# gwall-ceres/HighRes-net

Hardware: AMD Instinct MI355X
Metric: SR frames/sec (384x384 out) at B=32, n_views=32 (higher is better)
Workload: dtype bf16

## Files before the change

### highres-net_amd/hrnet_hip/csrc/common.h

```cpp
#pragma once
#include <hip/hip_runtime.h>
#include <stdint.h>
#include <stddef.h>
#include "prof.h"

#define HRN_F32 0
#define HRN_BF16 1
#define HRN_BF16X3 2

typedef __attribute__((ext_vector_type(8))) __bf16 bf16x8;
typedef __attribute__((ext_vector_type(4))) float f32x4;
typedef __attribute__((ext_vector_type(16))) float f32x16;
typedef __attribute__((ext_vector_type(4))) unsigned u32x4;
typedef __attribute__((ext_vector_type(2))) unsigned u32x2;

void hrn_set_error(const char* fmt, ...);
int hrn_allow_lds(const void* kernel, int bytes);
int hrn_device_cus(void);
#define HRN_CHECK(cond, code, ...)                                \
    do {                                                          \
        if (!(cond)) { hrn_set_error(__VA_ARGS__); return (code); } \
    } while (0)
#define HRN_HIP(call)                                                                    \
    do {                                                                                 \
        hipError_t e_ = (call);                                                          \
        if (e_ != hipSuccess) {                                                          \
            hrn_set_error("%s failed: %s (%s:%d)", #call, hipGetErrorString(e_), __FILE__, __LINE__); \
            return -5;                                                                   \
        }                                                                                \
    } while (0)
#define HRN_LAUNCH_CHECK()  HRN_HIP(hipGetLastError())

__device__ __forceinline__ float bf16_bits_to_f32(unsigned short b) {
    return __uint_as_float(((unsigned)b) << 16);
}
__device__ __forceinline__ unsigned short f32_to_bf16_bits(float f) {
    __bf16 h = (__bf16)f;
    return __builtin_bit_cast(unsigned short, h);
}
__device__ __forceinline__ unsigned pack2_bf16(float lo, float hi) {
    typedef __bf16 bf16x2_t __attribute__((ext_vector_type(2)));
    typedef float f32x2_t __attribute__((ext_vector_type(2)));
    const f32x2_t v = {lo, hi};
    return __builtin_bit_cast(unsigned, __builtin_convertvector(v, bf16x2_t));
}
__device__ __forceinline__ void split2_bf16(float a, float b, unsigned& hi, unsigned& lo) {
    hi = pack2_bf16(a, b);
    lo = pack2_bf16(a - __uint_as_float(hi << 16), b - __uint_as_float(hi & 0xffff0000u));
}

__device__ __forceinline__ void quad_transpose(u32x4 (&x)[4], bool b0, bool b1) {
#pragma unroll
    for (int d = 0; d < 4; ++d) {
#pragma unroll
        for (int p = 0; p < 4; p += 2) {
            const unsigned a = x[p][d], b = x[p + 1][d];
            const unsigned ra = (unsigned)__builtin_amdgcn_update_dpp(0, (int)b, 0xB1, 0xF, 0xF, true);
            const unsigned rb = (unsigned)__builtin_amdgcn_update_dpp(0, (int)a, 0xB1, 0xF, 0xF, true);
            x[p][d] = b0 ? ra : a;
            x[p + 1][d] = b0 ? b : rb;
        }
#pragma unroll
        for (int p = 0; p < 2; ++p) {
            const unsigned a = x[p][d], b = x[p + 2][d];
            const unsigned ra = (unsigned)__builtin_amdgcn_update_dpp(0, (int)b, 0x4E, 0xF, 0xF, true);
            const unsigned rb = (unsigned)__builtin_amdgcn_update_dpp(0, (int)a, 0x4E, 0xF, 0xF, true);
            x[p][d] = b1 ? ra : a;
            x[p + 2][d] = b1 ? b : rb;
        }
    }
}

template <int DT> struct ElemOf;
template <> struct ElemOf<HRN_F32>  { typedef float type;          static constexpr int size = 4; };
template <> struct ElemOf<HRN_BF16> { typedef unsigned short type; static constexpr int size = 2; };

template <int DT> __device__ __forceinline__ float load_elem(const void* p, size_t i);
template <> __device__ __forceinline__ float load_elem<HRN_F32>(const void* p, size_t i) { return ((const float*)p)[i]; }
template <> __device__ __forceinline__ float load_elem<HRN_BF16>(const void* p, size_t i) { return bf16_bits_to_f32(((const unsigned short*)p)[i]); }

template <int DT> __device__ __forceinline__ void store_elem(void* p, size_t i, float v);
template <> __device__ __forceinline__ void store_elem<HRN_F32>(void* p, size_t i, float v) { ((float*)p)[i] = v; }
template <> __device__ __forceinline__ void store_elem<HRN_BF16>(void* p, size_t i, float v) { ((unsigned short*)p)[i] = f32_to_bf16_bits(v); }

template <int DT> __device__ __forceinline__ f32x4 load4(const void* p, size_t i);
template <> __device__ __forceinline__ f32x4 load4<HRN_F32>(const void* p, size_t i) {
    return *(const f32x4*)((const float*)p + i);
}
template <> __device__ __forceinline__ f32x4 load4<HRN_BF16>(const void* p, size_t i) {
    uint2 u = *(const uint2*)((const unsigned short*)p + i);
    f32x4 r;
    r[0] = __uint_as_float(u.x << 16); r[1] = __uint_as_float(u.x & 0xffff0000u);
    r[2] = __uint_as_float(u.y << 16); r[3] = __uint_as_float(u.y & 0xffff0000u);
    return r;
}
template <int DT> __device__ __forceinline__ void store4(void* p, size_t i, f32x4 v);
template <> __device__ __forceinline__ void store4<HRN_F32>(void* p, size_t i, f32x4 v) {
    *(f32x4*)((float*)p + i) = v;
}
template <> __device__ __forceinline__ void store4<HRN_BF16>(void* p, size_t i, f32x4 v) {
    uint2 u; u.x = pack2_bf16(v[0], v[1]); u.y = pack2_bf16(v[2], v[3]);
    *(uint2*)((unsigned short*)p + i) = u;
}

template <int ST> __device__ __forceinline__ f32x4 act_ld4(const void* p, size_t lo, size_t i4) {
    if constexpr (ST == HRN_BF16X3) {
        const u32x2 h = __builtin_nontemporal_load((const u32x2*)p + i4);
        const u32x2 l = __builtin_nontemporal_load((const u32x2*)((const unsigned char*)p + lo) + i4);
        f32x4 r;
        r[0] = __uint_as_float(h[0] << 16) + __uint_as_float(l[0] << 16);
        r[1] = __uint_as_float(h[0] & 0xffff0000u) + __uint_as_float(l[0] & 0xffff0000u);
        r[2] = __uint_as_float(h[1] << 16) + __uint_as_float(l[1] << 16);
        r[3] = __uint_as_float(h[1] & 0xffff0000u) + __uint_as_float(l[1] & 0xffff0000u);
        return r;
    } else if constexpr (ST == HRN_BF16) {
        const u32x2 h = __builtin_nontemporal_load((const u32x2*)p + i4);
        return f32x4{__uint_as_float(h[0] << 16), __uint_as_float(h[0] & 0xffff0000u), __uint_as_float(h[1] << 16),
                     __uint_as_float(h[1] & 0xffff0000u)};
    } else {
        static_assert(ST == HRN_F32, "storage kind");
        return __builtin_nontemporal_load((const f32x4*)p + i4);
    }
}
template <int ST> __device__ __forceinline__ void act_st4(void* p, size_t lo, size_t i4, f32x4 v) {
    if constexpr (ST == HRN_BF16X3) {
        unsigned h0, l0, h1, l1;
        split2_bf16(v[0], v[1], h0, l0);
        split2_bf16(v[2], v[3], h1, l1);
        const u32x2 h = {h0, h1}, l = {l0, l1};
        __builtin_nontemporal_store(h, (u32x2*)p + i4);
        __builtin_nontemporal_store(l, (u32x2*)((unsigned char*)p + lo) + i4);
    } else if constexpr (ST == HRN_BF16) {
        const u32x2 h = {pack2_bf16(v[0], v[1]), pack2_bf16(v[2], v[3])};
        __builtin_nontemporal_store(h, (u32x2*)p + i4);
    } else {
        static_assert(ST == HRN_F32, "storage kind");
        __builtin_nontemporal_store(v, (f32x4*)p + i4);
    }
}
template <int ST> __device__ __forceinline__ float act_ld1(const void* p, size_t lo, size_t i) {
    if constexpr (ST == HRN_BF16X3) return bf16_bits_to_f32(((const unsigned short*)p)[i]) + bf16_bits_to_f32(((const unsigned short*)((const unsigned char*)p + lo))[i]);
    else if constexpr (ST == HRN_BF16) return bf16_bits_to_f32(((const unsigned short*)p)[i]);
    else return ((const float*)p)[i];
}

#define HRN_LAUNCH_ST(dt, KERNEL, ...)                                                                   \
    do {                                                                                                 \
        if ((dt) == HRN_BF16X3) hipLaunchKernelGGL(KERNEL<HRN_BF16X3>, __VA_ARGS__);                     \
        else if ((dt) == HRN_BF16) hipLaunchKernelGGL(KERNEL<HRN_BF16>, __VA_ARGS__);                    \
        else hipLaunchKernelGGL(KERNEL<HRN_F32>, __VA_ARGS__);                                           \
    } while (0)

__device__ __forceinline__ void block_pair_sum(const double* __restrict__ partial, int nblk, int C, double& s, double& ss) {
    __shared__ double red_ps[2][1024];
    const int c = (int)threadIdx.x % C, ph = (int)threadIdx.x / C, nph = (int)blockDim.x / C;
    double a = 0.0, b = 0.0;
#pragma unroll 4
    for (int k = ph; k < nblk; k += nph) { a += partial[((size_t)k * C + c) * 2]; b += partial[((size_t)k * C + c) * 2 + 1]; }
    red_ps[0][threadIdx.x] = a; red_ps[1][threadIdx.x] = b;
    __syncthreads();
    if (ph == 0)
        for (int k = 1; k < nph; ++k) { a += red_ps[0][k * C + c]; b += red_ps[1][k * C + c]; }
    s = a; ss = b;
}

static inline size_t hrn_align_up(size_t x, size_t a) { return (x + a - 1) / a * a; }
static inline int hrn_esize(int dt) { return dt == HRN_BF16 ? 2 : 4; }
static inline bool hrn_scale_ok(int s) { return s >= 2 && s <= 4; }
```

### highres-net_amd/hrnet_hip/csrc/conv3x3_r64.hip

```cpp
#include <type_traits>
#include "conv3x3.h"

namespace {

constexpr int HALO_H = CONV_TILE_H + 2;
constexpr int HALO_W = CONV_TILE_W + 2;
constexpr int IN_BYTES = HALO_H * HALO_W * 128;
constexpr int W_BYTES = 9 * 64 * 128;
constexpr int LDS_BYTES = W_BYTES + 2 * IN_BYTES + 256;

__device__ __forceinline__ void lds_done_then_barrier() {
    asm volatile("s_waitcnt lgkmcnt(0)" ::: "memory");
    __builtin_amdgcn_s_barrier();
    asm volatile("" ::: "memory");
}

__device__ __forceinline__ float raw_max(float a, float b) {
    float y;
    asm("v_max_f32 %0, %1, %2" : "=v"(y) : "v"(a), "v"(b));
    return y;
}

__device__ __attribute__((aligned(16))) unsigned hrn_r64_zero16[4];

template <bool RES>
__global__ __launch_bounds__(512, 2) void conv3x3_r64_kernel(const ConvParams p) {
    if (p.only_if_nonpos && p.only_if_nonpos[0] > 0.f) return;
    extern __shared__ __attribute__((aligned(16))) unsigned char smem[];
    unsigned char* w_lds = smem;
    float* bias_lds = (float*)(smem + W_BYTES + 2 * IN_BYTES);

    const int tid = threadIdx.x;
    const int lane = tid & 63;
    const int wave = __builtin_amdgcn_readfirstlane(tid >> 6);
    const int team = wave >> 2, tw = wave & 3;
    unsigned char* in_lds = smem + W_BYTES + team * IN_BYTES;
    const int r = lane & 31, hh = lane >> 5;
    const int H = p.H, W = p.W;
    const size_t hw = (size_t)H * W;
    const unsigned tiles_x = (W + CONV_TILE_W - 1) / CONV_TILE_W;
    const unsigned tiles_y = (H + CONV_TILE_H - 1) / CONV_TILE_H;
    const unsigned tiles = tiles_x * tiles_y;
    const unsigned total = tiles * (unsigned)p.M;
    const unsigned G = gridDim.x;
    const unsigned bid = blockIdx.x;
    const unsigned slot = (G & 7) == 0 ? (bid & 7) * (G >> 3) + (bid >> 3) : bid;
    if (slot >= total) return;
    const int ntl = (int)((total - slot + G - 1) / G);
    const int nmine = (ntl + 1 - team) >> 1;

    unsigned cur_m = (slot + team * G) / tiles, cur_t = (slot + team * G) - cur_m * tiles;
    const unsigned step_m = (2 * G) / tiles, step_t = 2 * G - step_m * tiles;

    {
        const u32x4* wg = (const u32x4*)p.wpk;
#pragma unroll
        for (int j = 0; j < W_BYTES / 16 / 512; ++j) {
            const int idx = tid + j * 512;
            const int row = idx >> 3, c = idx & 7;
            *(u32x4*)(w_lds + row * 128 + ((c ^ ((row >> 1) & 7)) << 4)) = wg[idx];
        }
        if (tid < 64) bias_lds[tid] = p.bias[tid];
    }

    unsigned voff[11], cm_lo = 0, cm_hi = 0;
    if (!RES) {
#pragma unroll
        for (int jj = 0; jj < 11; ++jj) {
            const int j = tw + 4 * jj;
            const int pix = j * 8 + (lane >> 3);
            const int py = pix / HALO_W, px = pix - py * HALO_W;
            voff[jj] = (unsigned)((py * W + px) * 128 + (((lane & 7) ^ ((pix >> 1) & 7)) << 4));
            unsigned cls = (py == 0 ? 1u : 0u) | (py == HALO_H - 1 ? 2u : 0u) | (px == 0 ? 4u : 0u) | (px == HALO_W - 1 ? 8u : 0u);
            if (pix >= HALO_H * HALO_W) cls = 0;
            if (jj < 8) cm_lo |= cls << (4 * jj); else cm_hi |= cls << (4 * (jj - 8));
        }
    }
    unsigned pend_F = 0;
    auto issue = [&](unsigned m, unsigned t) __attribute__((always_inline)) {
        const int ty = t / tiles_x;
        const int y0 = ty * CONV_TILE_H, x0 = (t - ty * tiles_x) * CONV_TILE_W;
        const unsigned char* base = (const unsigned char*)p.in + (size_t)m * hw * 128;
        const bool fast = !RES && y0 + CONV_TILE_H <= H && x0 + CONV_TILE_W <= W && (m > 0 || y0 > 0) &&
                          ((int)m + 1 < p.M || (size_t)(y0 + CONV_TILE_H) * W + x0 + CONV_TILE_W < hw);
        pend_F = 0;
        if (fast) {
            const unsigned char* hb = base + ((long)(y0 - 1) * W + (x0 - 1)) * 128;
#pragma unroll
            for (int jj = 0; jj < 11; ++jj) {
                const int j = tw + 4 * jj;
                if (j < 43) {
                    if (jj < 10 || j * 8 + (lane >> 3) < HALO_H * HALO_W)
                        __builtin_amdgcn_global_load_lds((const __attribute__((address_space(1))) void*)(hb + voff[jj]),
                                                         (__attribute__((address_space(3))) void*)(in_lds + j * 1024), 16, 0, 0);
                }
            }
            pend_F = (y0 == 0 ? 1u : 0u) | (y0 + CONV_TILE_H == H ? 2u : 0u) | (x0 == 0 ? 4u : 0u) | (x0 + CONV_TILE_W == W ? 8u : 0u);
            __builtin_amdgcn_sched_barrier(0);
            return;
        }
        int lq = lane;
        asm volatile("" : "+v"(lq));
#pragma unroll
        for (int jj = 0; jj < 11; ++jj) {
            const int j = tw + 4 * jj;
            if (j < 43) {
                const int pix = j * 8 + (lq >> 3);
                const int lc = (lq & 7) ^ ((pix >> 1) & 7);
                const int py = pix / HALO_W, px = pix - py * HALO_W;
                const int gy = y0 - 1 + py, gx = x0 - 1 + px;
                const bool ok = (unsigned)gy < (unsigned)H && (unsigned)gx < (unsigned)W;
                const unsigned char* src = ok ? base + (unsigned)((gy * W + gx) * 128 + lc * 16) : (const unsigned char*)hrn_r64_zero16;
                if (pix < HALO_H * HALO_W)
                    __builtin_amdgcn_global_load_lds((const __attribute__((address_space(1))) void*)src,
                                                     (__attribute__((address_space(3))) void*)(in_lds + j * 1024), 16, 0, 0);
            }
        }
        __builtin_amdgcn_sched_barrier(0);
    };
    auto fix_borders = [&]() __attribute__((always_inline)) {
        if (!RES && pend_F) {
            const unsigned fm = pend_F * 0x11111111u;
            const unsigned hit_lo = cm_lo & fm, hit_hi = cm_hi & fm;
            const u32x4 z = {0u, 0u, 0u, 0u};
#pragma unroll
            for (int jj = 0; jj < 11; ++jj) {
                const int j = tw + 4 * jj;
                if (j < 43) {
                    const unsigned h = jj < 8 ? (hit_lo >> (4 * jj)) & 15u : (hit_hi >> (4 * (jj - 8))) & 15u;
                    if (h) *(u32x4*)(in_lds + j * 1024 + lane * 16) = z;
                }
            }
        }
    };

    const bool has_slope = p.slope != nullptr;
    const float slope = has_slope ? p.slope[0] : 0.f;
    const bool slope01 = slope >= 0.f && slope <= 1.f;
    const unsigned lds0 = (unsigned)(__UINTPTR_TYPE__)(__attribute__((address_space(3))) unsigned char*)smem;
    unsigned a_off[4], a_off_hi[4], b_off[4][3];
#pragma unroll
    for (int ks = 0; ks < 4; ++ks) {
        a_off[ks] = lds0 + r * 128 + (((ks * 2 + hh) ^ ((r >> 1) & 7)) << 4);
        a_off_hi[ks] = a_off[ks] + 4 * 8192;
    }
#pragma unroll
    for (int row = 0; row < 4; ++row)
#pragma unroll
        for (int kx = 0; kx < 3; ++kx) {
            const int pix = (2 * tw + row) * HALO_W + r + kx;
            b_off[row][kx] = lds0 + (unsigned)(W_BYTES + team * IN_BYTES) + (((unsigned)pix << 7) | ((unsigned)(((pix >> 1) & 7) ^ hh) << 4));
        }

    f32x16 acc[2][2];

    auto multiply = [&]() __attribute__((always_inline)) {
#pragma unroll
        for (int cb = 0; cb < 2; ++cb)
#pragma unroll
            for (int g = 0; g < 4; ++g) {
                const f32x4 b = *(const f32x4*)(bias_lds + cb * 32 + 8 * g + 4 * hh);
#pragma unroll
                for (int j = 0; j < 4; ++j) { acc[cb][0][4 * g + j] = b[j]; acc[cb][1][4 * g + j] = b[j]; }
            }
        constexpr int NK = 36;
        bf16x8 fa[3][2], fb[3][2];
        auto rd = [&](bf16x8& dst, unsigned addr, int imm) __attribute__((always_inline)) {
            asm volatile("ds_read_b128 %0, %1 offset:%2" : "=v"(dst) : "v"(addr), "n"(imm));
        };
        auto load_part = [&](int i, int part) __attribute__((always_inline)) {
            const int s_ = i % 3, tap = i >> 2, ks = i & 3;
            const int ky = tap / 3, kx = tap - ky * 3;
            if (part < 2) {
                rd(fa[s_][part], tap < 4 ? a_off[ks] : a_off_hi[ks], (tap < 4 ? tap : tap - 4) * 8192 + part * 4096);
            } else {
                unsigned kbits = 0;
                if (ks) asm volatile("s_mov_b32 %0, %1" : "=s"(kbits) : "n"(ks << 5));
                rd(fb[s_][part - 2], b_off[part - 2 + ky][kx] ^ kbits, 0);
            }
        };
        asm volatile("s_waitcnt lgkmcnt(0)" ::: "memory");
        __builtin_amdgcn_s_setprio(3);
#pragma unroll
        for (int i = 0; i < 2; ++i)
#pragma unroll
            for (int part = 0; part < 4; ++part) load_part(i, part);
        __builtin_amdgcn_sched_barrier(0);
#pragma unroll
        for (int i = 0; i < NK; ++i) {
            const int s_ = i % 3;
            const bool more = i + 2 < NK;
            if (i < NK - 1) asm volatile("s_waitcnt lgkmcnt(5)" : "+v"(fa[s_][0]), "+v"(fb[s_][0]));
            else asm volatile("s_waitcnt lgkmcnt(1)" : "+v"(fa[s_][0]), "+v"(fb[s_][0]));
            acc[0][0] = __builtin_amdgcn_mfma_f32_32x32x16_bf16(fa[s_][0], fb[s_][0], acc[0][0], 0, 0, 0);
            if (more) load_part(i + 2, 0);
            __builtin_amdgcn_sched_barrier(0);
            if (more) asm volatile("s_waitcnt lgkmcnt(5)" : "+v"(fb[s_][1]));
            else if (i == NK - 2) asm volatile("s_waitcnt lgkmcnt(4)" : "+v"(fb[s_][1]));
            else asm volatile("s_waitcnt lgkmcnt(0)" : "+v"(fb[s_][1]));
            acc[0][1] = __builtin_amdgcn_mfma_f32_32x32x16_bf16(fa[s_][0], fb[s_][1], acc[0][1], 0, 0, 0);
            if (more) load_part(i + 2, 1);
            __builtin_amdgcn_sched_barrier(0);
            asm volatile("" : "+v"(fa[s_][1]));
            acc[1][0] = __builtin_amdgcn_mfma_f32_32x32x16_bf16(fa[s_][1], fb[s_][0], acc[1][0], 0, 0, 0);
            if (more) load_part(i + 2, 2);
            __builtin_amdgcn_sched_barrier(0);
            acc[1][1] = __builtin_amdgcn_mfma_f32_32x32x16_bf16(fa[s_][1], fb[s_][1], acc[1][1], 0, 0, 0);
            if (more) load_part(i + 2, 3);
            __builtin_amdgcn_sched_barrier(0);
        }
        __builtin_amdgcn_s_setprio(0);
    };

    u32x4 resv[2][4];
    float res_alpha = 1.f;
    auto fetch_residual = [&]() __attribute__((always_inline)) {
        const int m = (int)cur_m;
        const int ty = cur_t / tiles_x;
        const int y0 = ty * CONV_TILE_H, x0 = (cur_t - ty * tiles_x) * CONV_TILE_W;
        const unsigned char* rbase = (const unsigned char*)p.res + (size_t)m * hw * 128;
        if (p.res_mode == 3) {
            const int ob = m / p.out_h, oi = m - ob * p.out_h;
            rbase = (const unsigned char*)p.res + ((size_t)ob * p.res_vs + oi) * hw * 128;
            res_alpha = p.alphas ? p.alphas[(size_t)ob * p.alpha_vs + (p.pair_last - oi)] : 1.f;
        }
#pragma unroll
        for (int pb = 0; pb < 2; ++pb) {
            const int gy = y0 + 2 * tw + pb, gyc = gy < H ? gy : H - 1;
#pragma unroll
            for (int j = 0; j < 4; ++j) {
                const int gxj = x0 + (r & ~3) + j, gxjc = gxj < W ? gxj : W - 1;
                resv[pb][j] = __builtin_nontemporal_load((const u32x4*)(rbase + (unsigned)((gyc * W + gxjc) * 128 + hh * 64 + (r & 3) * 16)));
            }
        }
    };

    auto finish = [&](bool more) __attribute__((always_inline)) {
        const int m = (int)cur_m;
        const int ty = cur_t / tiles_x;
        const int y0 = ty * CONV_TILE_H, x0 = (cur_t - ty * tiles_x) * CONV_TILE_W;
        cur_t += step_t; cur_m += step_m;
        if (cur_t >= tiles) { cur_t -= tiles; ++cur_m; }
        size_t oimg = (size_t)m;
        int ob = 0, oi = 0;
        if (p.out_h > 0) { ob = m / p.out_h; oi = m - ob * p.out_h; oimg = (size_t)ob * p.out_vs + oi; }
        unsigned char* outp = (unsigned char*)p.out + (oimg * hw + (size_t)y0 * W + x0) * 128;
        if (RES) {
#pragma unroll
            for (int pb = 0; pb < 2; ++pb)
#pragma unroll
                for (int g = 0; g < 4; ++g) asm volatile("" :: "v"(resv[pb][g]));
            asm volatile("" :: "v"(res_alpha));
        }
        if (more) issue(cur_m, cur_t);
        auto epilogue = [&](auto act_c) __attribute__((always_inline)) {
        constexpr int ACT = decltype(act_c)::value;
#pragma unroll
        for (int pb = 0; pb < 2; ++pb) {
            const int gy = y0 + 2 * tw + pb;
            u32x4 uu[4];
            if (RES) quad_transpose(resv[pb], (lane & 1) != 0, (lane & 2) != 0);
#pragma unroll
            for (int g = 0; g < 4; ++g) {
                float xa[4], xb[4];
#pragma unroll
                for (int j = 0; j < 4; ++j) { xa[j] = acc[0][pb][4 * g + j]; xb[j] = acc[1][pb][4 * g + j]; }
                if (ACT == 1) {
#pragma unroll
                    for (int j = 0; j < 4; ++j) { xa[j] = raw_max(xa[j], slope * xa[j]); xb[j] = raw_max(xb[j], slope * xb[j]); }
                } else if (ACT == 2) {
#pragma unroll
                    for (int j = 0; j < 4; ++j) { xa[j] = xa[j] >= 0.f ? xa[j] : slope * xa[j]; xb[j] = xb[j] >= 0.f ? xb[j] : slope * xb[j]; }
                }
                u32x4 u;
                if (RES) {
                    float v[8];
#pragma unroll
                    for (int j = 0; j < 4; ++j) {
                        const u32x2 sw = __builtin_amdgcn_permlane32_swap(__float_as_uint(xa[j]), __float_as_uint(xb[j]), false, false);
                        v[j] = __uint_as_float(sw[0]);
                        v[4 + j] = __uint_as_float(sw[1]);
                    }
                    const u32x4 rq = resv[pb][g];
#pragma unroll
                    for (int j = 0; j < 4; ++j) {
                        const float r0 = __uint_as_float(rq[j] << 16), r1 = __uint_as_float(rq[j] & 0xffff0000u);
                        if (p.res_mode == 3) { v[2 * j] = r0 + res_alpha * v[2 * j]; v[2 * j + 1] = r1 + res_alpha * v[2 * j + 1]; }
                        else { v[2 * j] += r0; v[2 * j + 1] += r1; }
                    }
#pragma unroll
                    for (int j = 0; j < 4; ++j) u[j] = pack2_bf16(v[2 * j], v[2 * j + 1]);
                } else {
                    const u32x2 s0 = __builtin_amdgcn_permlane32_swap(pack2_bf16(xa[0], xa[1]), pack2_bf16(xb[0], xb[1]), false, false);
                    const u32x2 s1 = __builtin_amdgcn_permlane32_swap(pack2_bf16(xa[2], xa[3]), pack2_bf16(xb[2], xb[3]), false, false);
                    u[0] = s0[0]; u[1] = s1[0]; u[2] = s0[1]; u[3] = s1[1];
                }
                uu[g] = u;
            }
            {
                quad_transpose(uu, (lane & 1) != 0, (lane & 2) != 0);
                unsigned char* oq = outp + (unsigned)(((2 * tw + pb) * W + (r & ~3)) * 128 + hh * 64 + (r & 3) * 16);
#pragma unroll
                for (int j = 0; j < 4; ++j)
                    if (gy < H && x0 + (r & ~3) + j < W) __builtin_nontemporal_store(uu[j], (u32x4*)(oq + j * 128));
            }
        }
        };
        if (!has_slope) epilogue(std::integral_constant<int, 0>{});
        else if (slope01) epilogue(std::integral_constant<int, 1>{});
        else epilogue(std::integral_constant<int, 2>{});
        {
            const int nst = 4 * ((y0 + 2 * tw < H) + (y0 + 2 * tw + 1 < H));
            if (nst == 8) asm volatile("s_waitcnt vmcnt(8)" ::: "memory");
            else if (nst == 4) asm volatile("s_waitcnt vmcnt(4)" ::: "memory");
            else asm volatile("s_waitcnt vmcnt(0)" ::: "memory");
        }
        fix_borders();
    };

    if (nmine > 0) issue(cur_m, cur_t);
    asm volatile("s_waitcnt vmcnt(0)" ::: "memory");
    fix_borders();
    lds_done_then_barrier();

    for (int ph = 0; ph <= ntl; ++ph) {
        const int q = ph - team;
        if (q >= 0) {
            const int k = q >> 1;
            if (k < nmine) {
                if ((q & 1) == 0) { if (RES) fetch_residual(); multiply(); }
                else finish(k + 1 < nmine);
            }
        }
        if (ph < ntl) lds_done_then_barrier();
    }
}


template <bool RES>
int launch_r64(const ConvParams& p, long grid, hipStream_t stream) {
    { const int rc_lds = hrn_allow_lds((const void*)conv3x3_r64_kernel<RES>, LDS_BYTES); if (rc_lds) return rc_lds; }
    hipLaunchKernelGGL(conv3x3_r64_kernel<RES>, dim3((unsigned)grid), dim3(512), LDS_BYTES, stream, p);
    HRN_LAUNCH_CHECK();
    return 0;
}

}

int hrn_launch_conv3x3_r64(const ConvParams& p, hipStream_t stream) {
    if (p.scale || p.relu || p.in_pair || p.res_mode == 2) return -100;
    static_assert(LDS_BYTES <= 160 * 1024, "LDS budget");
    const long tiles = (long)((p.W + CONV_TILE_W - 1) / CONV_TILE_W) * ((p.H + CONV_TILE_H - 1) / CONV_TILE_H);
    const long total = tiles * p.M;
    HRN_CHECK(total > 0, -2, "conv3x3_r64: bad tile count %ld", total);
    if (total >= (1L << 30) || (long)p.H * p.W * 128 >= (1L << 31)) return -100;
    long grid = hrn_device_cus();
    if (total < grid) grid = total;
    if (grid >= 8) grid &= ~7L;
    const double px = (double)p.M * p.H * p.W;
    HrnProfScope prof(p.res_mode ? "conv3x3_bf16_64x64+res" : "conv3x3_bf16_64x64", 2.0 * 64 * 64 * 9 * px,
                      px * 2 * (64 + 64 + (p.res_mode ? 64 : 0)), stream);
    return p.res_mode ? launch_r64<true>(p, grid, stream) : launch_r64<false>(p, grid, stream);
}
```

Baseline: 2000.

## Switch r64 conv from 32x32x16 to 16x16x32 MFMA with new LDS swizzle

Rewrites the 64-channel 3x3 conv inner loop to use 16x16x32 bf16 MFMAs with a 4x4 accumulator grid instead of 32x32x16 with 2x2. It introduces a new LDS swizzle layout header, permutes the weight rows so each lane's accumulator maps to four channels, and reorders the pipelined ds_read/waitcnt schedule. The epilogue replaces the quad transposes and permlane32 swaps with a single DPP pair exchange, and the residual loads are adjusted to match. The aim is cheaper epilogue shuffles and different LDS bank behaviour, at the cost of more MFMA instructions and more LDS reads per K step.

```diff
diff --git a/highres-net_amd/hrnet_hip/csrc/common.h b/highres-net_amd/hrnet_hip/csrc/common.h
--- a/highres-net_amd/hrnet_hip/csrc/common.h
+++ b/highres-net_amd/hrnet_hip/csrc/common.h
@@ -47,28 +47,6 @@
 __device__ __forceinline__ void split2_bf16(float a, float b, unsigned& hi, unsigned& lo) {
     hi = pack2_bf16(a, b);
     lo = pack2_bf16(a - __uint_as_float(hi << 16), b - __uint_as_float(hi & 0xffff0000u));
-}
-
-__device__ __forceinline__ void quad_transpose(u32x4 (&x)[4], bool b0, bool b1) {
-#pragma unroll
-    for (int d = 0; d < 4; ++d) {
-#pragma unroll
-        for (int p = 0; p < 4; p += 2) {
-            const unsigned a = x[p][d], b = x[p + 1][d];
-            const unsigned ra = (unsigned)__builtin_amdgcn_update_dpp(0, (int)b, 0xB1, 0xF, 0xF, true);
-            const unsigned rb = (unsigned)__builtin_amdgcn_update_dpp(0, (int)a, 0xB1, 0xF, 0xF, true);
-            x[p][d] = b0 ? ra : a;
-            x[p + 1][d] = b0 ? b : rb;
-        }
-#pragma unroll
-        for (int p = 0; p < 2; ++p) {
-            const unsigned a = x[p][d], b = x[p + 2][d];
-            const unsigned ra = (unsigned)__builtin_amdgcn_update_dpp(0, (int)b, 0x4E, 0xF, 0xF, true);
-            const unsigned rb = (unsigned)__builtin_amdgcn_update_dpp(0, (int)a, 0x4E, 0xF, 0xF, true);
-            x[p][d] = b1 ? ra : a;
-            x[p + 2][d] = b1 ? b : rb;
-        }
-    }
 }
 
 template <int DT> struct ElemOf;
diff --git a/highres-net_amd/hrnet_hip/csrc/conv3x3_r64.hip b/highres-net_amd/hrnet_hip/csrc/conv3x3_r64.hip
--- a/highres-net_amd/hrnet_hip/csrc/conv3x3_r64.hip
+++ b/highres-net_amd/hrnet_hip/csrc/conv3x3_r64.hip
@@ -1,5 +1,6 @@
 #include <type_traits>
 #include "conv3x3.h"
+#include "r64_layout.h"
 
 namespace {
 
@@ -19,6 +20,13 @@
     float y;
     asm("v_max_f32 %0, %1, %2" : "=v"(y) : "v"(a), "v"(b));
     return y;
+}
+
+__device__ __forceinline__ void pair_exchange(unsigned a_e0, unsigned a_e1, bool odd, unsigned& lo, unsigned& hi) {
+    const unsigned send = odd ? a_e0 : a_e1;
+    const unsigned recv = (unsigned)__builtin_amdgcn_update_dpp(0, (int)send, 0xB1, 0xF, 0xF, true);
+    lo = odd ? recv : a_e0;
+    hi = odd ? a_e1 : recv;
 }
 
 __device__ __attribute__((aligned(16))) unsigned hrn_r64_zero16[4];
@@ -35,7 +43,7 @@
     const int wave = __builtin_amdgcn_readfirstlane(tid >> 6);
     const int team = wave >> 2, tw = wave & 3;
     unsigned char* in_lds = smem + W_BYTES + team * IN_BYTES;
-    const int r = lane & 31, hh = lane >> 5;
+    const int c15 = lane & 15, q = lane >> 4;
     const int H = p.H, W = p.W;
     const size_t hw = (size_t)H * W;
     const unsigned tiles_x = (W + CONV_TILE_W - 1) / CONV_TILE_W;
@@ -58,7 +66,7 @@
         for (int j = 0; j < W_BYTES / 16 / 512; ++j) {
             const int idx = tid + j * 512;
             const int row = idx >> 3, c = idx & 7;
-            *(u32x4*)(w_lds + row * 128 + ((c ^ ((row >> 1) & 7)) << 4)) = wg[idx];
+            *(u32x4*)(w_lds + r64_chunk_off(r64_w_row(row >> 6, row & 63), c)) = wg[idx];
         }
         if (tid < 64) bias_lds[tid] = p.bias[tid];
     }
@@ -70,7 +78,7 @@
             const int j = tw + 4 * jj;
             const int pix = j * 8 + (lane >> 3);
             const int py = pix / HALO_W, px = pix - py * HALO_W;
-            voff[jj] = (unsigned)((py * W + px) * 128 + (((lane & 7) ^ ((pix >> 1) & 7)) << 4));
+            voff[jj] = (unsigned)((py * W + px) * 128 + (r64_dma_chunk(j, lane) << 4));
             unsigned cls = (py == 0 ? 1u : 0u) | (py == HALO_H - 1 ? 2u : 0u) | (px == 0 ? 4u : 0u) | (px == HALO_W - 1 ? 8u : 0u);
             if (pix >= HALO_H * HALO_W) cls = 0;
             if (jj < 8) cm_lo |= cls << (4 * jj); else cm_hi |= cls << (4 * (jj - 8));
@@ -106,7 +114,7 @@
             const int j = tw + 4 * jj;
             if (j < 43) {
                 const int pix = j * 8 + (lq >> 3);
-                const int lc = (lq & 7) ^ ((pix >> 1) & 7);
+                const int lc = r64_dma_chunk(j, lq);
                 const int py = pix / HALO_W, px = pix - py * HALO_W;
                 const int gy = y0 - 1 + py, gx = x0 - 1 + px;
                 const bool ok = (unsigned)gy < (unsigned)H && (unsigned)gx < (unsigned)W;
@@ -138,81 +146,78 @@
     const float slope = has_slope ? p.slope[0] : 0.f;
     const bool slope01 = slope >= 0.f && slope <= 1.f;
     const unsigned lds0 = (unsigned)(__UINTPTR_TYPE__)(__attribute__((address_space(3))) unsigned char*)smem;
-    unsigned a_off[4], a_off_hi[4], b_off[4][3];
-#pragma unroll
-    for (int ks = 0; ks < 4; ++ks) {
-        a_off[ks] = lds0 + r * 128 + (((ks * 2 + hh) ^ ((r >> 1) & 7)) << 4);
-        a_off_hi[ks] = a_off[ks] + 4 * 8192;
+    unsigned a_off[2], a_off_hi[2], b_off[4][3];
+#pragma unroll
+    for (int kh = 0; kh < 2; ++kh) {
+        a_off[kh] = lds0 + (unsigned)r64_frag_off(0, c15, q, kh);
+        a_off_hi[kh] = a_off[kh] + 4 * 8192;
     }
 #pragma unroll
     for (int row = 0; row < 4; ++row)
 #pragma unroll
-        for (int kx = 0; kx < 3; ++kx) {
-            const int pix = (2 * tw + row) * HALO_W + r + kx;
-            b_off[row][kx] = lds0 + (unsigned)(W_BYTES + team * IN_BYTES) + (((unsigned)pix << 7) | ((unsigned)(((pix >> 1) & 7) ^ hh) << 4));
-        }
-
-    f32x16 acc[2][2];
+        for (int kx = 0; kx < 3; ++kx)
+            b_off[row][kx] = lds0 + (unsigned)(W_BYTES + team * IN_BYTES) + (unsigned)r64_frag_off((2 * tw + row) * HALO_W + kx, c15, q, 0);
+
+    f32x4 acc[4][4];
 
     auto multiply = [&]() __attribute__((always_inline)) {
-#pragma unroll
-        for (int cb = 0; cb < 2; ++cb)
-#pragma unroll
-            for (int g = 0; g < 4; ++g) {
-                const f32x4 b = *(const f32x4*)(bias_lds + cb * 32 + 8 * g + 4 * hh);
-#pragma unroll
-                for (int j = 0; j < 4; ++j) { acc[cb][0][4 * g + j] = b[j]; acc[cb][1][4 * g + j] = b[j]; }
-            }
-        constexpr int NK = 36;
-        bf16x8 fa[3][2], fb[3][2];
+        {
+            const f32x4 b = *(const f32x4*)(bias_lds + r64_acc_channel(c15, 0));
+#pragma unroll
+            for (int cb = 0; cb < 4; ++cb)
+#pragma unroll
+                for (int pxb = 0; pxb < 4; ++pxb) acc[cb][pxb] = f32x4{b[cb], b[cb], b[cb], b[cb]};
+        }
+        constexpr int NK = 18;
+        bf16x8 fa[3][4], fb[3][4];
         auto rd = [&](bf16x8& dst, unsigned addr, int imm) __attribute__((always_inline)) {
             asm volatile("ds_read_b128 %0, %1 offset:%2" : "=v"(dst) : "v"(addr), "n"(imm));
         };
         auto load_part = [&](int i, int part) __attribute__((always_inline)) {
-            const int s_ = i % 3, tap = i >> 2, ks = i & 3;
+            const int s_ = i % 3, tap = i >> 1, kh = i & 1;
             const int ky = tap / 3, kx = tap - ky * 3;
-            if (part < 2) {
-                rd(fa[s_][part], tap < 4 ? a_off[ks] : a_off_hi[ks], (tap < 4 ? tap : tap - 4) * 8192 + part * 4096);
+            if (part < 4) {
+                unsigned kbits = 0;
+                if (kh) asm volatile("s_mov_b32 %0, %1" : "=s"(kbits) : "n"(64));
+                rd(fb[s_][part], b_off[(part >> 1) + ky][kx] ^ kbits, (part & 1) * 2048);
             } else {
-                unsigned kbits = 0;
-                if (ks) asm volatile("s_mov_b32 %0, %1" : "=s"(kbits) : "n"(ks << 5));
-                rd(fb[s_][part - 2], b_off[part - 2 + ky][kx] ^ kbits, 0);
-            }
+                rd(fa[s_][part - 4], tap < 4 ? a_off[kh] : a_off_hi[kh], (tap < 4 ? tap : tap - 4) * 8192 + (part - 4) * 2048);
+            }
+        };
+        auto wait_lgkm = [&](int n, bf16x8& f) __attribute__((always_inline)) {
+            asm volatile("s_waitcnt lgkmcnt(%1)" : "+v"(f) : "n"(n));
         };
         asm volatile("s_waitcnt lgkmcnt(0)" ::: "memory");
         __builtin_amdgcn_s_setprio(3);
 #pragma unroll
-        for (int i = 0; i < 2; ++i)
-#pragma unroll
-            for (int part = 0; part < 4; ++part) load_part(i, part);
+        for (int part = 0; part < 8; ++part) load_part(0, part);
+#pragma unroll
+        for (int part = 0; part < 4; ++part) load_part(1, part);
+        asm volatile("s_waitcnt lgkmcnt(11)" ::: "memory");
+#pragma unroll
+        for (int part = 4; part < 8; ++part) load_part(1, part);
         __builtin_amdgcn_sched_barrier(0);
 #pragma unroll
         for (int i = 0; i < NK; ++i) {
             const int s_ = i % 3;
             const bool more = i + 2 < NK;
-            if (i < NK - 1) asm volatile("s_waitcnt lgkmcnt(5)" : "+v"(fa[s_][0]), "+v"(fb[s_][0]));
-            else asm volatile("s_waitcnt lgkmcnt(1)" : "+v"(fa[s_][0]), "+v"(fb[s_][0]));
-            acc[0][0] = __builtin_amdgcn_mfma_f32_32x32x16_bf16(fa[s_][0], fb[s_][0], acc[0][0], 0, 0, 0);
-            if (more) load_part(i + 2, 0);
-            __builtin_amdgcn_sched_barrier(0);
-            if (more) asm volatile("s_waitcnt lgkmcnt(5)" : "+v"(fb[s_][1]));
-            else if (i == NK - 2) asm volatile("s_waitcnt lgkmcnt(4)" : "+v"(fb[s_][1]));
-            else asm volatile("s_waitcnt lgkmcnt(0)" : "+v"(fb[s_][1]));
-            acc[0][1] = __builtin_amdgcn_mfma_f32_32x32x16_bf16(fa[s_][0], fb[s_][1], acc[0][1], 0, 0, 0);
-            if (more) load_part(i + 2, 1);
-            __builtin_amdgcn_sched_barrier(0);
-            asm volatile("" : "+v"(fa[s_][1]));
-            acc[1][0] = __builtin_amdgcn_mfma_f32_32x32x16_bf16(fa[s_][1], fb[s_][0], acc[1][0], 0, 0, 0);
-            if (more) load_part(i + 2, 2);
-            __builtin_amdgcn_sched_barrier(0);
-            acc[1][1] = __builtin_amdgcn_mfma_f32_32x32x16_bf16(fa[s_][1], fb[s_][1], acc[1][1], 0, 0, 0);
-            if (more) load_part(i + 2, 3);
-            __builtin_amdgcn_sched_barrier(0);
+#pragma unroll
+            for (int g = 0; g < 4; ++g) {
+                const int younger = (3 - g) + (i + 1 < NK ? 8 : 0) + (more ? 2 * g : 0);
+                if (g == 0) asm volatile("" : "+v"(fb[s_][0]), "+v"(fb[s_][1]), "+v"(fb[s_][2]), "+v"(fb[s_][3]));
+                wait_lgkm(younger < 13 ? younger : 13, fa[s_][g]);
+#pragma unroll
+                for (int pxb = 0; pxb < 4; ++pxb) {
+                    acc[g][pxb] = __builtin_amdgcn_mfma_f32_16x16x32_bf16(fb[s_][pxb], fa[s_][g], acc[g][pxb], 0, 0, 0);
+                    if (more && (pxb & 1) == 0) load_part(i + 2, 2 * g + (pxb >> 1));
+                    __builtin_amdgcn_sched_barrier(0);
+                }
+            }
         }
         __builtin_amdgcn_s_setprio(0);
     };
 
-    u32x4 resv[2][4];
+    u32x4 resv[4][2];
     float res_alpha = 1.f;
     auto fetch_residual = [&]() __attribute__((always_inline)) {
         const int m = (int)cur_m;
@@ -225,12 +230,12 @@
             res_alpha = p.alphas ? p.alphas[(size_t)ob * p.alpha_vs + (p.pair_last - oi)] : 1.f;
         }
 #pragma unroll
-        for (int pb = 0; pb < 2; ++pb) {
-            const int gy = y0 + 2 * tw + pb, gyc = gy < H ? gy : H - 1;
-#pragma unroll
-            for (int j = 0; j < 4; ++j) {
-                const int gxj = x0 + (r & ~3) + j, gxjc = gxj < W ? gxj : W - 1;
-                resv[pb][j] = __builtin_nontemporal_load((const u32x4*)(rbase + (unsigned)((gyc * W + gxjc) * 128 + hh * 64 + (r & 3) * 16)));
+        for (int pxb = 0; pxb < 4; ++pxb) {
+            const int gy = y0 + 2 * tw + (pxb >> 1), gyc = gy < H ? gy : H - 1;
+#pragma unroll
+            for (int h = 0; h < 2; ++h) {
+                const int gx = x0 + 16 * (pxb & 1) + 4 * q + 2 * h + (lane & 1), gxc = gx < W ? gx : W - 1;
+                resv[pxb][h] = __builtin_nontemporal_load((const u32x4*)(rbase + (unsigned)((gyc * W + gxc) * 128 + (c15 >> 1) * 16)));
             }
         }
     };
@@ -247,41 +252,43 @@
         unsigned char* outp = (unsigned char*)p.out + (oimg * hw + (size_t)y0 * W + x0) * 128;
         if (RES) {
 #pragma unroll
-            for (int pb = 0; pb < 2; ++pb)
-#pragma unroll
-                for (int g = 0; g < 4; ++g) asm volatile("" :: "v"(resv[pb][g]));
+            for (int pxb = 0; pxb < 4; ++pxb)
+#pragma unroll
+                for (int h = 0; h < 2; ++h) asm volatile("" :: "v"(resv[pxb][h]));
             asm volatile("" :: "v"(res_alpha));
         }
         if (more) issue(cur_m, cur_t);
+        const bool odd = (lane & 1) != 0;
+        const int lane_px = 4 * q + (lane & 1);
+        const unsigned lane_off = (unsigned)(lane_px * 128 + (c15 >> 1) * 16);
         auto epilogue = [&](auto act_c) __attribute__((always_inline)) {
         constexpr int ACT = decltype(act_c)::value;
 #pragma unroll
-        for (int pb = 0; pb < 2; ++pb) {
-            const int gy = y0 + 2 * tw + pb;
-            u32x4 uu[4];
-            if (RES) quad_transpose(resv[pb], (lane & 1) != 0, (lane & 2) != 0);
-#pragma unroll
-            for (int g = 0; g < 4; ++g) {
-                float xa[4], xb[4];
-#pragma unroll
-                for (int j = 0; j < 4; ++j) { xa[j] = acc[0][pb][4 * g + j]; xb[j] = acc[1][pb][4 * g + j]; }
+        for (int pxb = 0; pxb < 4; ++pxb) {
+            const int gy = y0 + 2 * tw + (pxb >> 1);
+#pragma unroll
+            for (int h = 0; h < 2; ++h) {
+                float xe[4], xo[4];
+#pragma unroll
+                for (int cb = 0; cb < 4; ++cb) { xe[cb] = acc[cb][pxb][2 * h]; xo[cb] = acc[cb][pxb][2 * h + 1]; }
                 if (ACT == 1) {
 #pragma unroll
-                    for (int j = 0; j < 4; ++j) { xa[j] = raw_max(xa[j], slope * xa[j]); xb[j] = raw_max(xb[j], slope * xb[j]); }
+                    for (int cb = 0; cb < 4; ++cb) { xe[cb] = raw_max(xe[cb], slope * xe[cb]); xo[cb] = raw_max(xo[cb], slope * xo[cb]); }
                 } else if (ACT == 2) {
 #pragma unroll
-                    for (int j = 0; j < 4; ++j) { xa[j] = xa[j] >= 0.f ? xa[j] : slope * xa[j]; xb[j] = xb[j] >= 0.f ? xb[j] : slope * xb[j]; }
+                    for (int cb = 0; cb < 4; ++cb) { xe[cb] = xe[cb] >= 0.f ? xe[cb] : slope * xe[cb]; xo[cb] = xo[cb] >= 0.f ? xo[cb] : slope * xo[cb]; }
                 }
                 u32x4 u;
                 if (RES) {
                     float v[8];
 #pragma unroll
-                    for (int j = 0; j < 4; ++j) {
-                        const u32x2 sw = __builtin_amdgcn_permlane32_swap(__float_as_uint(xa[j]), __float_as_uint(xb[j]), false, false);
-                        v[j] = __uint_as_float(sw[0]);
-                        v[4 + j] = __uint_as_float(sw[1]);
+                    for (int cb = 0; cb < 4; ++cb) {
+                        unsigned lo, hi;
+                        pair_exchange(__float_as_uint(xe[cb]), __float_as_uint(xo[cb]), odd, lo, hi);
+                        v[cb] = __uint_as_float(lo);
+                        v[4 + cb] = __uint_as_float(hi);
                     }
-                    const u32x4 rq = resv[pb][g];
+                    const u32x4 rq = resv[pxb][h];
 #pragma unroll
                     for (int j = 0; j < 4; ++j) {
                         const float r0 = __uint_as_float(rq[j] << 16), r1 = __uint_as_float(rq[j] & 0xffff0000u);
@@ -291,18 +298,13 @@
 #pragma unroll
                     for (int j = 0; j < 4; ++j) u[j] = pack2_bf16(v[2 * j], v[2 * j + 1]);
                 } else {
-                    const u32x2 s0 = __builtin_amdgcn_permlane32_swap(pack2_bf16(xa[0], xa[1]), pack2_bf16(xb[0], xb[1]), false, false);
-                    const u32x2 s1 = __builtin_amdgcn_permlane32_swap(pack2_bf16(xa[2], xa[3]), pack2_bf16(xb[2], xb[3]), false, false);
-                    u[0] = s0[0]; u[1] = s1[0]; u[2] = s0[1]; u[3] = s1[1];
-                }
-                uu[g] = u;
-            }
-            {
-                quad_transpose(uu, (lane & 1) != 0, (lane & 2) != 0);
-                unsigned char* oq = outp + (unsigned)(((2 * tw + pb) * W + (r & ~3)) * 128 + hh * 64 + (r & 3) * 16);
-#pragma unroll
-                for (int j = 0; j < 4; ++j)
-                    if (gy < H && x0 + (r & ~3) + j < W) __builtin_nontemporal_store(uu[j], (u32x4*)(oq + j * 128));
+                    unsigned lo0, hi0, lo1, hi1;
+                    pair_exchange(pack2_bf16(xe[0], xe[1]), pack2_bf16(xo[0], xo[1]), odd, lo0, hi0);
+                    pair_exchange(pack2_bf16(xe[2], xe[3]), pack2_bf16(xo[2], xo[3]), odd, lo1, hi1);
+                    u[0] = lo0; u[1] = lo1; u[2] = hi0; u[3] = hi1;
+                }
+                unsigned char* oq = outp + ((unsigned)(((2 * tw + (pxb >> 1)) * W + 16 * (pxb & 1) + 2 * h) * 128) + lane_off);
+                if (gy < H && x0 + 16 * (pxb & 1) + 2 * h + lane_px < W) __builtin_nontemporal_store(u, (u32x4*)oq);
             }
         }
         };
@@ -310,7 +312,7 @@
         else if (slope01) epilogue(std::integral_constant<int, 1>{});
         else epilogue(std::integral_constant<int, 2>{});
         {
-            const int nst = 4 * ((y0 + 2 * tw < H) + (y0 + 2 * tw + 1 < H));
+            const int nst = x0 + CONV_TILE_W <= W ? 4 * ((y0 + 2 * tw < H) + (y0 + 2 * tw + 1 < H)) : 0;
             if (nst == 8) asm volatile("s_waitcnt vmcnt(8)" ::: "memory");
             else if (nst == 4) asm volatile("s_waitcnt vmcnt(4)" ::: "memory");
             else asm volatile("s_waitcnt vmcnt(0)" ::: "memory");
@@ -324,11 +326,11 @@
     lds_done_then_barrier();
 
     for (int ph = 0; ph <= ntl; ++ph) {
-        const int q = ph - team;
-        if (q >= 0) {
-            const int k = q >> 1;
+        const int s = ph - team;
+        if (s >= 0) {
+            const int k = s >> 1;
             if (k < nmine) {
-                if ((q & 1) == 0) { if (RES) fetch_residual(); multiply(); }
+                if ((s & 1) == 0) { if (RES) fetch_residual(); multiply(); }
                 else finish(k + 1 < nmine);
             }
         }
diff --git a/highres-net_amd/hrnet_hip/csrc/r64_layout.h b/highres-net_amd/hrnet_hip/csrc/r64_layout.h
--- /dev/null
+++ b/highres-net_amd/hrnet_hip/csrc/r64_layout.h
@@ -0,0 +1,16 @@
+#pragma once
+
+#if defined(__HIPCC__)
+#define R64_FN __host__ __device__ inline constexpr
+#else
+#define R64_FN inline constexpr
+#endif
+
+R64_FN int r64_swz(int row) { return row & 7; }
+R64_FN int r64_chunk_off(int row, int chunk) { return row * 128 + ((chunk ^ r64_swz(row)) << 4); }
+R64_FN int r64_frag_chunk(int q, int kh) { return kh * 4 + q; }
+R64_FN int r64_frag_off(int base_row, int c15, int q, int kh) { return r64_chunk_off(base_row + c15, r64_frag_chunk(q, kh)); }
+R64_FN int r64_dma_pixel(int piece, int lane) { return piece * 8 + (lane >> 3); }
+R64_FN int r64_dma_chunk(int piece, int lane) { return (lane & 7) ^ r64_swz(r64_dma_pixel(piece, lane)); }
+R64_FN int r64_w_row(int tap, int cout) { return tap * 64 + (cout & 3) * 16 + (cout >> 2); }
+R64_FN int r64_acc_channel(int c15, int cb) { return 4 * c15 + cb; }
```

New measurement: 2086 (median of 6 runs). 1.04x the previous value.
